# psipred/merizo_search

Hardware: AMD Instinct MI355X
Metric: queries/sec, exact 128-d cosine top-10 (recall@10 vs brute force = 1.0000) (higher is better)
Workload: dtype f32

## Files before the change

### merizo_search_amd/csrc/ms_scan_pf16.h

```cpp
#pragma once
#include "ms_scan_pf.h"

typedef _Float16 f16x8 __attribute__((ext_vector_type(8)));
constexpr uint32_t MS_PF16_MAGIC = 0x3631464du;
#define MS_PF_ERR_F16X2 5.5e-4f
#define MS_PF_ERR_F16X1 1.05e-3f

template <int KL, int NW, bool SAMPLE, bool MASK, int NQP>
__global__ __launch_bounds__(64 * NW, NW / 4) void ms_scan_pf16_kernel(const ScanParams p) {
    static_assert(NQP == 1 || NQP == 2, "query parts");
    static_assert(NW == 4 || NW == 8, "one or two waves per SIMD");
    constexpr int PPW = 16 / NW;
#ifdef MS_STAMP
    const unsigned long long tl_entry = __builtin_amdgcn_s_memrealtime();
    unsigned long long tl_setup = 0, tl_first = 0, tl_loop = 0;
#endif
    if (ms_gate_closed(p.gate, p.gate_epoch)) return;
    extern __shared__ __attribute__((aligned(16))) char smem[];
    typedef __attribute__((address_space(3))) char lds_char_t;
    typedef volatile __attribute__((address_space(3))) uint32_t lds_flag_t;
    typedef __attribute__((address_space(3))) ms_u32x2 lds_cand_t;
    const int tid = threadIdx.x, lane = tid & 63;
    const int wave = __builtin_amdgcn_readfirstlane(tid >> 6);
    const int r = lane & 31, h = lane >> 5;
    lds_flag_t *arrived = (lds_flag_t *)((lds_char_t *)smem + PF2_OFF_CNT);
    const float *auxring = reinterpret_cast<const float *>(smem + PF2_OFF_AUX);

    const int bid = blockIdx.x;
    const int per_super = 8 * p.n_qgroups;
    const int super = bid / per_super, within = bid % per_super;
    const int stream = super * 8 + (within & 7);
    const int qg = within >> 3;
    if (stream >= p.n_streams) return;
    const int64_t row_begin = (int64_t)stream * p.rows_per_stream;
    const int64_t row_end = (row_begin + p.rows_per_stream < p.n) ? row_begin + p.rows_per_stream : p.n;
    const int nfull = (int)((row_end - row_begin) >> 6);
    const int rem = (int)((row_end - row_begin) & 63);
    const int ntl = SAMPLE ? (nfull < p.max_tiles ? nfull : p.max_tiles) : nfull + (rem > 0 ? 1 : 0);
    constexpr bool mask_on = MASK;

    const int qtile = qg * NW + wave;
    const bool has_q = qtile < p.n_qtiles;
    if (tid < PF2_ARR) arrived[tid] = 0u;
    __syncthreads();
    const uint32_t ring_lds = __builtin_amdgcn_readfirstlane((uint32_t)(uintptr_t)(lds_char_t *)smem);

    const uint32_t voff = (uint32_t)(16 * lane);
    const uint64_t img0 = (uint64_t)(uintptr_t)p.pf_image + (uint64_t)(row_begin >> 6) * 16384u + (uint32_t)(1024 * PPW) * (uint32_t)wave;
    uint64_t it_sb = 0;
    uint32_t it_dst = 0;
    auto issue_prep = [&](int t) __attribute__((always_inline)) {
        const uint64_t b = img0 + (uint64_t)t * 16384u;
        const uint32_t b_lo = (uint32_t)__builtin_amdgcn_readfirstlane((uint32_t)b);
        const uint32_t b_hi = (uint32_t)__builtin_amdgcn_readfirstlane((uint32_t)(b >> 32));
        it_sb = ((uint64_t)b_hi << 32) | (uint64_t)b_lo;
        it_dst = (uint32_t)__builtin_amdgcn_readfirstlane(ring_lds + (uint32_t)(t % PF2_R) * 16384u + (uint32_t)(1024 * PPW) * (uint32_t)wave);
    };
    auto issue_piece = [&](auto i_c) __attribute__((always_inline)) {
        constexpr int I = decltype(i_c)::value;
        if constexpr (I < PPW) {
            const uint32_t d = (uint32_t)__builtin_amdgcn_readfirstlane(it_dst);
            const uint32_t lo = (uint32_t)__builtin_amdgcn_readfirstlane((uint32_t)it_sb), hi = (uint32_t)__builtin_amdgcn_readfirstlane((uint32_t)(it_sb >> 32));
            ms_glds_s16<1024 * I>(d + 1024 * I, voff, ((uint64_t)hi << 32) | (uint64_t)lo);
        }
    };
    auto issue_aux = [&](int t) __attribute__((always_inline)) {
        if constexpr (MASK) {
            int64_t row = row_begin + (int64_t)t * 64 + lane;
            if (row >= p.n) row = p.n - 1;
            const uint32_t dst = wave == 0 ? ring_lds + PF2_OFF_AUX + (uint32_t)(t % PF2_AUXR) * 256u
                                           : ring_lds + PF2_OFF_DUMMY + (uint32_t)(wave - 1) * 256u;
// ... 21 lines not shown
    auto read_arrived = [&](int t) __attribute__((always_inline)) { seen = arrived[t & (PF2_ARR - 1)]; };
    auto wait_arrived = [&](int t) __attribute__((always_inline)) {
        const uint32_t need = (uint32_t)NW * (uint32_t)(t / PF2_ARR + 1);
        uint32_t sv_, spins_, av_;
        static_assert(PF2_ARR == 16, "the mask below");
        asm volatile("s_waitcnt lgkmcnt(0)\n\t"
                     "v_readfirstlane_b32 %0, %2\n\t"
                     "s_cmp_ge_u32 %0, %5\n\t"
                     "s_setprio 2\n\t"
                     "s_cbranch_scc1 2f\n\t"
                     "s_setprio 0\n\t"
                     "s_and_b32 %0, %4, 15\n\t"
                     "s_lshl_b32 %0, %0, 2\n\t"
                     "s_add_u32 %0, %0, %6\n\t"
                     "v_mov_b32 %3, %0\n\t"
                     "s_mov_b32 %1, 0\n\t"
                     "1:\n\t"
                     "s_sleep 1\n\t"
                     "ds_read_b32 %2, %3\n\t"
                     "s_add_u32 %1, %1, 1\n\t"
                     "s_waitcnt lgkmcnt(0)\n\t"
                     "v_readfirstlane_b32 %0, %2\n\t"
                     "s_cmp_ge_u32 %0, %5\n\t"
                     "s_cbranch_scc1 2f\n\t"
                     "s_cmp_lt_u32 %1, 0x1000000\n\t"
                     "s_cbranch_scc1 1b\n\t"
                     "s_trap 2\n\t"
                     "2:"
                     : "=&s"(sv_), "=&s"(spins_), "+v"(seen), "=&v"(av_) : "s"(t), "s"(need), "s"(arr_lds) : "memory", "scc");
        asm volatile("" ::: "memory");
    };
    const int qidx = qtile * 32 + r;
    const bool q_valid = qidx < p.nq;
    const bool hist_on = !SAMPLE && p.hist != nullptr && p.lb_s != nullptr;
    f32x4 qv[16];
    float pre_lb = -INFINITY, pre_stp = 0.0f, pre_qlen = 0.0f;
    uint32_t pre_magic = MS_PF16_MAGIC, pre_n = (uint32_t)p.n;
    int pre_sr = 0;
    if (has_q) {
        const uint32_t *trailer = reinterpret_cast<const uint32_t *>(reinterpret_cast<const char *>(p.pf_image) + (size_t)((p.n + 63) >> 6) * 16384u);
        pre_magic = trailer[0];
        pre_sr = (int)trailer[1];
        pre_n = trailer[2];
        const f32x4 *src = reinterpret_cast<const f32x4 *>(p.qn + (size_t)(q_valid ? qidx : 0) * MS_DIM + 64 * h);
#pragma unroll
        for (int i = 0; i < 16; ++i) qv[i] = src[i];
        if (!SAMPLE && p.lb_s != nullptr) pre_lb = p.lb_s[qidx];
        if (hist_on && q_valid) pre_stp = p.hstep[qidx];
        if (MASK && p.qlen != nullptr && q_valid) pre_qlen = p.qlen[qidx];
    }
    asm volatile("" ::: "memory");
#pragma unroll
    for (int t = 0; t < PF2_D; ++t)
        if (t < ntl) issue_tile(t);

    if (!has_q) {
        if (ntl > 0) {
            if (ntl >= PF2_D) wait_own(std::integral_constant<int, PF2_D - PF2_W>{}); else ms_pf2_vmcnt<0>();
#pragma unroll
            for (int t = 0; t < PF2_W; ++t)
                if (t < ntl) publish(t);
        }
        for (int t = 0; t < ntl; ++t) {
            if (t + 1 < ntl) { read_arrived(t + 1); wait_arrived(t + 1); }
            if (t + PF2_D < ntl) {
                issue_tile(t + PF2_D);
                wait_own(std::integral_constant<int, PF2_D - PF2_W>{});
            } else {
                ms_pf2_vmcnt<0>();
            }
            if (t + PF2_W < ntl) publish(t + PF2_W);
        }
        return;
    }

    ScanState<SAMPLE ? 1 : KL> st;
    ScanHist hg;
    f16x8 qh[8], ql[NQP == 2 ? 8 : 1];
#pragma unroll
    for (int j = 0; j < (SAMPLE ? 1 : KL); ++j) { st.ls[j] = -INFINITY; st.li[j] = MS_IDX_NONE; }
    st.floor = -INFINITY;
    st.tau = -INFINITY;
    if (!SAMPLE && p.lb_s != nullptr) {
        const float lb = pre_lb;
        st.floor = (lb == -INFINITY) ? -INFINITY : nextafterf(lb, -INFINITY);
        st.tau = st.floor;
    }
    if (!q_valid) { st.floor = INFINITY; st.tau = INFINITY; }
    if (!SAMPLE && (p.debug_flags & 1)) { st.floor = INFINITY; st.tau = INFINITY; }
    hg.counters = nullptr; hg.base = 0.0f; hg.step = 0.0f; hg.inv_step = 0.0f;
    if (hist_on && q_valid) {
        const float stp = pre_stp, lb = pre_lb;
        if (stp > 0.0f && lb > -INFINITY) { hg.counters = p.hist + (size_t)qidx * 16; hg.base = lb; hg.step = stp; hg.inv_step = 1.0f / stp; }
    }
    float up = 1.0f, down = 1.0f;
    {
        const uint32_t magic = (uint32_t)__builtin_amdgcn_readfirstlane((int)pre_magic);
        const int sr = __builtin_amdgcn_readfirstlane(pre_sr);
        const uint32_t img_n = (uint32_t)__builtin_amdgcn_readfirstlane((int)pre_n);
        if (magic != MS_PF16_MAGIC || img_n != (uint32_t)p.n) __builtin_trap();
        f32x4 v[16];
        float m = 0.0f;
        float rinv = 1.0f;
        if (p.qraw_eps > 0.0f) {
            float ss = 0.0f;
#pragma unroll
            for (int i = 0; i < 16; ++i) { ss += qv[i].x * qv[i].x; ss += qv[i].y * qv[i].y; ss += qv[i].z * qv[i].z; ss += qv[i].w * qv[i].w; }
            ss = ss + ms_xor32_f(ss, h);
            rinv = 1.0f / fmaxf(sqrtf(ss), p.qraw_eps);
        }
#pragma unroll
        for (int i = 0; i < 16; ++i) {
            v[i] = q_valid ? qv[i] * rinv : f32x4{0.0f, 0.0f, 0.0f, 0.0f};
            m = fmaxf(m, fmaxf(fmaxf(fabsf(v[i].x), fabsf(v[i].y)), fmaxf(fabsf(v[i].z), fabsf(v[i].w))));
        }
        m = fmaxf(m, ms_xor32_f(m, h));
        int sq = 0;
        if (m > 0.0f && m < INFINITY) sq = 13 - ((int)((__float_as_uint(m) >> 23) & 0xFFu) - 127);
        sq = sq > 60 ? 60 : (sq < -60 ? -60 : sq);
        const float qs = __uint_as_float((uint32_t)(127 + sq) << 23);
        up = __uint_as_float((uint32_t)(127 + sr + sq) << 23);
        down = __uint_as_float((uint32_t)(127 - sr - sq) << 23);
#pragma unroll
        for (int b = 0; b < 8; ++b) {
            const f32x4 a0 = v[2 * b] * qs, a1 = v[2 * b + 1] * qs;
            const float x[8] = {a0.x, a0.y, a0.z, a0.w, a1.x, a1.y, a1.z, a1.w};
#pragma unroll
            for (int j = 0; j < 8; ++j) {
                const float c = fminf(fmaxf(x[j], -65504.0f), 65504.0f);
                const _Float16 hi16 = (_Float16)c;
                qh[b][j] = hi16;
                if constexpr (NQP == 2) ql[b][j] = (_Float16)(c - (float)hi16);
            }
        }
    }
    float tau_s = st.tau * up;
    const float my_qlen = (mask_on && p.qlen != nullptr && q_valid) ? pre_qlen : 0.0f;
    const float qlen_eff = mask_on ? my_qlen : INFINITY;
    const float mincov_eff = mask_on ? p.mincov : 0.0f;
    float smax = -INFINITY;
    auto apply_mask = [&](f32x16 &acc, int t, int half) __attribute__((always_inline)) {
        const f32x4 *ax = reinterpret_cast<const f32x4 *>(auxring + (t & (PF2_AUXR - 1)) * 64 + 32 * half + 4 * h);
#pragma unroll
        for (int g = 0; g < 4; ++g) {
            const f32x4 len4 = ax[2 * g];
#pragma unroll
            for (int j = 0; j < 4; ++j) {
                const float mk = (qlen_eff >= len4[j] * mincov_eff) ? 1.0f : 0.0f;
                acc[4 * g + j] = acc[4 * g + j] * mk;
            }
        }
    };
    bool neg_tau = !SAMPLE && mask_on && (__ballot(st.tau < 0.0f) != 0);
    const bool pace_on = !SAMPLE && p.prog != nullptr;
    constexpr int PACE_LEAD = 48;
    int pace_left = 16384;
    auto pace = [&](int t) __attribute__((always_inline)) {
        if (wave != 0 || (t & 15) != 0) return;
        const uint64_t line = (uint64_t)(uintptr_t)(p.prog + (size_t)stream * 16);
        const uint32_t l_lo = (uint32_t)__builtin_amdgcn_readfirstlane((uint32_t)line), l_hi = (uint32_t)__builtin_amdgcn_readfirstlane((uint32_t)(line >> 32));
        const uint64_t sline = ((uint64_t)l_hi << 32) | (uint64_t)l_lo;
        const uint32_t tag = p.prog_epoch << 24;
        if (lane == 0) __hip_atomic_store(p.prog + (size_t)stream * 16 + qg, tag | (uint32_t)t, __ATOMIC_RELAXED, __HIP_MEMORY_SCOPE_AGENT);
        if (t < PACE_LEAD) return;
        typedef uint32_t u32x16_ __attribute__((ext_vector_type(16)));
        for (; pace_left > 0; --pace_left) {
            u32x16_ w;
            asm volatile("s_load_dwordx16 %0, %1, 0x0 glc\n\ts_waitcnt lgkmcnt(0)" : "=s"(w) : "s"(sline) : "memory");
            uint32_t mn = 0xFFFFFFu;
#pragma unroll
            for (int i = 0; i < 16; ++i) {
                const uint32_t v = ((w[i] >> 24) == p.prog_epoch) ? (w[i] & 0xFFFFFFu) : 0u;
                if (i < p.n_qgroups) mn = v < mn ? v : mn;
            }
            if ((uint32_t)t <= mn + (uint32_t)PACE_LEAD) break;
            __builtin_amdgcn_s_sleep(64);
        }
    };
    auto retau = [&]() __attribute__((always_inline)) { tau_s = st.tau * up; };

    uint32_t ccnt = 0;
    auto cand_slot = [&](uint32_t c) __attribute__((always_inline)) -> lds_cand_t * {
        return (lds_cand_t *)((lds_char_t *)smem + PF2_OFF_CAND + (wave * PF2_CAND) * 512) + c * 64 + lane;
    };
    auto flush = [&]() __attribute__((always_inline)) {
        for (uint32_t c = 0; __ballot(ccnt > c) != 0; ++c) {
            const ms_u32x2 e = *cand_slot(c < PF2_CAND ? c : 0);
            const float v = (ccnt > c) ? __uint_as_float(e.x) : -INFINITY;
            ms_lane_insert<SAMPLE ? 1 : KL>(st, v, e.y, 0, h);
            ms_lane_insert<SAMPLE ? 1 : KL>(st, v, e.y, 1, h);
        }
        ccnt = 0;
        retau();
    };
    constexpr bool VISIT2 = !(MASK && (NQP == 2 || KL >= 16));
    auto visit_v2 = [&](f32x16 &sc_v, int t, int half, bool check_rows) __attribute__((always_inline)) {
        if (mask_on) apply_mask(sc_v, t, half);
        const uint32_t sub_row0 = (uint32_t)(row_begin + (int64_t)t * 64) + (uint32_t)(32 * half + 4 * h);
#pragma unroll 1
        for (;;) {
            bool ovf = false;
            float g0, g1, g2, g3;
            asm("v_max3_f32 %0, %4, %5, %6\n\tv_max3_f32 %1, %8, %9, %10\n\tv_max3_f32 %2, %12, %13, %14\n\tv_max3_f32 %3, %16, %17, %18\n\t"
                "v_max_f32 %0, %0, %7\n\tv_max_f32 %1, %1, %11\n\tv_max_f32 %2, %2, %15\n\tv_max_f32 %3, %3, %19"
                : "=&v"(g0), "=&v"(g1), "=&v"(g2), "=&v"(g3)
                : "v"(sc_v[0]), "v"(sc_v[1]), "v"(sc_v[2]), "v"(sc_v[3]), "v"(sc_v[4]), "v"(sc_v[5]), "v"(sc_v[6]), "v"(sc_v[7]), "v"(sc_v[8]),
                  "v"(sc_v[9]), "v"(sc_v[10]), "v"(sc_v[11]), "v"(sc_v[12]), "v"(sc_v[13]), "v"(sc_v[14]), "v"(sc_v[15]));
#define MS_PF16_REG(I)                                                                                                   \
            {                                                                                                            \
                const float ss = sc_v[I];                                                                                \
                const uint32_t row = sub_row0 + (uint32_t)(8 * ((I) >> 2) + ((I) & 3));                                    \
                bool pass = ss > tau_s;                                                                                  \
                if (check_rows) pass = pass && ((int64_t)row < row_end);                                                 \
                if (pass) {                                                                                              \
                    if (ccnt < (uint32_t)PF2_CAND) {                                                                     \
                        const float s_ = ss * down;                       \
                        if (hg.counters != nullptr) ms_hist_count(hg, s_);                                               \
                        *cand_slot(ccnt) = ms_u32x2{__float_as_uint(s_), row};                                           \
                        ccnt += 1;                                                                                       \
                        sc_v[I] = -INFINITY;                                                                             \
                    } else {                                                                                             \
                        ovf = true;                                                                                      \
                    }                                                                                                    \
// ... 42 lines not shown
            const uint32_t row = sub_row0 + (uint32_t)(8 * (i >> 2) + (i & 3));
            const float s = ss * down;
            bool pass = ss > tau_s;
            if (check_rows) pass = pass && ((int64_t)row < row_end);
            if (pass) {
                if (hg.counters != nullptr) ms_hist_count(hg, s);
                *cand_slot(ccnt) = ms_u32x2{__float_as_uint(s), row};
                ccnt += 1;
            }
            if (__builtin_expect(__ballot(ccnt >= PF2_CAND) != 0, 0)) flush();
        }
    };
    auto visit = [&](f32x16 &sc_v, int t, int half, bool check_rows) __attribute__((always_inline)) {
        if constexpr (VISIT2) visit_v2(sc_v, t, half, check_rows); else visit_v1(sc_v, t, half, check_rows);
    };

#ifdef MS_STAMP
    unsigned long long sp_t0 = 0, sp_sync = 0, sp_vis = 0, sp_nvis = 0, sp_chain = 0, sp_hist = 0, sp_lgkm = 0, sp_flow = 0;
#define PF2_T0() sp_t0 = __builtin_amdgcn_s_memtime()
#define PF2_ACC(V) { const unsigned long long now_ = __builtin_amdgcn_s_memtime(); V += now_ - sp_t0; sp_t0 = now_; }
#else
#define PF2_T0()
#define PF2_ACC(V)
#endif
    f32x4 fr[16];
    f32x16 acc0, acc1;
#pragma unroll
    for (int i = 0; i < 16; ++i) { acc0[i] = -INFINITY; acc1[i] = -INFINITY; }

    auto frag_base = [&](int t) __attribute__((always_inline)) -> const f32x4 * {
        return reinterpret_cast<const f32x4 *>(smem + (size_t)(t % PF2_R) * 16384 + 16 * lane);
    };
    auto filter = [&](int t, f32x16 &pv0, f32x16 &pv1) __attribute__((always_inline)) {
        if (SAMPLE) {
            if (mask_on && t > 0) { apply_mask(pv0, t - 1, 0); apply_mask(pv1, t - 1, 1); }
#pragma unroll
            for (int i = 0; i < 16; ++i) { smax = (pv0[i] > smax) ? pv0[i] : smax; smax = (pv1[i] > smax) ? pv1[i] : smax; }
        } else {
            float mx, mx1;
#define MS_PF16_MAX(M, PV)                                                                                                                        \
            asm("v_max3_f32 %0, %1, %2, %3\n\tv_max3_f32 %0, %0, %4, %5\n\tv_max3_f32 %0, %0, %6, %7\n\tv_max3_f32 %0, %0, %8, %9\n\t"             \
                "v_max3_f32 %0, %0, %10, %11\n\tv_max3_f32 %0, %0, %12, %13\n\tv_max3_f32 %0, %0, %14, %15\n\tv_max_f32 %0, %0, %16"               \
                : "=&v"(M) : "v"(PV[0]), "v"(PV[1]), "v"(PV[2]), "v"(PV[3]), "v"(PV[4]), "v"(PV[5]), "v"(PV[6]), "v"(PV[7]), "v"(PV[8]), "v"(PV[9]), \
                  "v"(PV[10]), "v"(PV[11]), "v"(PV[12]), "v"(PV[13]), "v"(PV[14]), "v"(PV[15]))
            MS_PF16_MAX(mx, pv0);
            MS_PF16_MAX(mx1, pv1);
#undef MS_PF16_MAX
            const bool hit0 = __ballot(mx > tau_s) != 0, hit1 = __ballot(mx1 > tau_s) != 0;
            if (__builtin_expect(hit0 || hit1 || neg_tau, 0)) {
                PF2_T0();
                if (t > 0) {
                    if (hit0 || neg_tau) visit(pv0, t - 1, 0, false);
                    if (hit1 || neg_tau) visit(pv1, t - 1, 1, false);
                }
                if (mask_on) neg_tau = __ballot(st.tau < 0.0f) != 0;
#ifdef MS_STAMP
                sp_nvis += 1;
#endif
                PF2_ACC(sp_vis)
            }
        }
    };
    auto stage = [&](auto steady_c, int t, f32x16 &out0, f32x16 &out1) __attribute__((always_inline)) {
        constexpr bool STEADY = decltype(steady_c)::value;
        PF2_T0();
        asm volatile("s_waitcnt lgkmcnt(0)" ::: "memory");
        PF2_ACC(sp_lgkm)
        if (STEADY || t + 1 < ntl) wait_arrived(t + 1);
        PF2_ACC(sp_sync)
        filter(t, out0, out1);
#pragma unroll
        for (int i = 0; i < 16; ++i) { out0[i] = 0.0f; out1[i] = 0.0f; }
        const f32x4 *src = frag_base(t + 1);
        const bool issuing = STEADY || t + PF2_D < ntl;
#define MS_PF2_BLOCK(B)                                                                                               \
        {                                                                                                             \
            const f16x8 f0 = __builtin_bit_cast(f16x8, fr[2 * (B)]), f1 = __builtin_bit_cast(f16x8, fr[2 * (B) + 1]);   \
            out0 = __builtin_amdgcn_mfma_f32_32x32x16_f16(f0, qh[B], out0, 0, 0, 0);                                  \
            out1 = __builtin_amdgcn_mfma_f32_32x32x16_f16(f1, qh[B], out1, 0, 0, 0);                                  \
            if constexpr (NQP == 2) {                                                                                 \
                out0 = __builtin_amdgcn_mfma_f32_32x32x16_f16(f0, ql[B], out0, 0, 0, 0);                              \
                out1 = __builtin_amdgcn_mfma_f32_32x32x16_f16(f1, ql[B], out1, 0, 0, 0);                              \
            }                                                                                                         \
            __builtin_amdgcn_sched_barrier(0);                                                                        \
            fr[2 * (B)] = src[64 * (2 * (B))];                                                                        \
            fr[2 * (B) + 1] = src[64 * (2 * (B) + 1)];                                                                \
        }
        MS_PF2_BLOCK(0)
        __builtin_amdgcn_sched_barrier(0);
        MS_PF2_BLOCK(1)
        if (STEADY || issuing) issue_prep(t + PF2_D);
        __builtin_amdgcn_sched_barrier(0);
        MS_PF2_BLOCK(2)
        if (STEADY || issuing) issue_piece(std::integral_constant<int, 0>{});
        __builtin_amdgcn_sched_barrier(0);
        MS_PF2_BLOCK(3)
        if (STEADY || issuing) issue_piece(std::integral_constant<int, 1>{});
        __builtin_amdgcn_sched_barrier(0);
        MS_PF2_BLOCK(4)
        if (STEADY || issuing) issue_piece(std::integral_constant<int, 2>{});
        __builtin_amdgcn_sched_barrier(0);
        MS_PF2_BLOCK(5)
        if (STEADY || issuing) { issue_piece(std::integral_constant<int, 3>{}); issue_aux(t + PF2_D); }
        __builtin_amdgcn_sched_barrier(0);
        MS_PF2_BLOCK(6)
        PF2_ACC(sp_chain)
        if (STEADY || issuing) wait_own(std::integral_constant<int, PF2_D - PF2_W>{}); else ms_pf2_vmcnt<0>();
        PF2_ACC(sp_flow)
        if (STEADY || t + PF2_W < ntl) publish(t + PF2_W);
        read_arrived(t + 2);
        __builtin_amdgcn_sched_barrier(0);
        MS_PF2_BLOCK(7)
#undef MS_PF2_BLOCK
#ifdef MS_STAMP
        asm volatile("s_nop 0" : "+v"(out0), "+v"(out1));
#endif
// ... 37 lines not shown
                PF2_T0();
                if (t - 1 + PF2_D < ntl) wait_own(std::integral_constant<int, 2>{}); else ms_pf2_vmcnt<0>();
                const ms_u32x4 *hp = reinterpret_cast<const ms_u32x4 *>(smem + PF2_OFF_HIST + hist_area * 2048 + r * 64);
                const ms_u32x4 c0 = hp[0], c1 = hp[1], c2 = hp[2], c3 = hp[3];
                const uint32_t c[16] = {c0.x, c0.y, c0.z, c0.w, c1.x, c1.y, c1.z, c1.w, c2.x, c2.y, c2.z, c2.w, c3.x, c3.y, c3.z, c3.w};
                uint32_t cum = 0;
                int n_lt = 0;
#pragma unroll
                for (int j = 15; j >= 0; --j) { cum += c[j]; n_lt += (cum < (uint32_t)p.k) ? 1 : 0; }
                const int J = 15 - n_lt;
                if (hg.counters != nullptr && J >= 1) {
                    st.floor = fmaxf(st.floor, ms_next_below(ms_hist_edge(hg, J)));
                    st.tau = fmaxf(st.tau, st.floor);
                }
                asm volatile("s_waitcnt lgkmcnt(0)" ::: "memory");
                retau();
                if (mask_on) neg_tau = __ballot(st.tau < 0.0f) != 0;
                PF2_ACC(sp_hist)
            }
        };
        int t = 0;
        for (; t + PF2_D < ntl; ++t) {
            if ((t & 1) == 0) {
                if (pace_on) pace(t);
                if (hist_on) hist_step(t);
            }
            stage(std::true_type{}, t, acc0, acc1);
        }
        for (; t < ntl; ++t) {
            if ((t & 1) == 0 && hist_on) hist_step(t);
            stage(std::false_type{}, t, acc0, acc1);
        }
#ifdef MS_STAMP
        if (!SAMPLE && lane == 0 && p.stamps != nullptr && (size_t)bid * 64 + 64 <= 4 * 4 * 65536) {
            unsigned long long *o = p.stamps + ((size_t)bid * 8 + wave) * 8;
            tl_loop = __builtin_amdgcn_s_memrealtime();
            o[0] = __builtin_amdgcn_s_memtime() - sp_c0;
            o[1] = __builtin_amdgcn_s_memrealtime() - sp_r0;
            o[2] = (unsigned long long)ntl;
            o[3] = (sp_lgkm << 32) | (sp_flow & 0xFFFFFFFFull);
            o[4] = sp_vis; o[5] = sp_nvis; o[6] = sp_chain; o[7] = (sp_hist << 32) | (sp_sync & 0xFFFFFFFFull);
        }
#endif
        if (pace_on && wave == 0 && lane == 0)
            __hip_atomic_store(p.prog + (size_t)stream * 16 + qg, (p.prog_epoch << 24) | 0xFFFFFFu, __ATOMIC_RELAXED, __HIP_MEMORY_SCOPE_AGENT);
        if (SAMPLE) {
            if (mask_on) { apply_mask(acc0, ntl - 1, 0); apply_mask(acc1, ntl - 1, 1); }
#pragma unroll
            for (int i = 0; i < 16; ++i) { smax = (acc0[i] > smax) ? acc0[i] : smax; smax = (acc1[i] > smax) ? acc1[i] : smax; }
        } else {
            visit(acc0, ntl - 1, 0, true);
            visit(acc1, ntl - 1, 1, true);
            flush();
        }
    }

    if (SAMPLE) {
        smax = smax * down;
        const float other = ms_xor32_f(smax, h);
        if (h == 0) {
            const float hi = (other > smax) ? other : smax, lo = (other > smax) ? smax : other;
            const size_t o = ((size_t)stream * p.nq_pad + qidx) * p.k;
            p.part_s[o] = hi;
            p.part_i[o] = (hi > -INFINITY) ? (uint32_t)(2 * stream) : MS_IDX_NONE;
            if (p.k > 1) {
                p.part_s[o + 1] = lo;
                p.part_i[o + 1] = (lo > -INFINITY) ? (uint32_t)(2 * stream + 1) : MS_IDX_NONE;
            }
        }
        return;
    }
#pragma unroll
    for (int j = 0; j < (SAMPLE ? 1 : KL); ++j) {
        const int rank = h * KL + j;
        if (rank < p.k) {
            const size_t o = ((size_t)stream * p.nq_pad + qidx) * p.k + rank;
            p.part_s[o] = st.ls[j];
            p.part_i[o] = st.li[j];
        }
    }
#ifdef MS_STAMP
    if (!SAMPLE && lane == 0 && p.stamps != nullptr && bid < 4096) {
        asm volatile("s_waitcnt vmcnt(0)" ::: "memory");
        unsigned long long *o = p.stamps + 8 * 8 * 4096 + ((size_t)bid * 8 + wave) * 8;
        o[0] = tl_entry; o[1] = tl_setup; o[2] = tl_first; o[3] = tl_loop; o[4] = __builtin_amdgcn_s_memrealtime();
    }
#endif
}

template <int KL, int NW, bool MASK, int NQP>
int launch_scan_pf16(const ScanPlan &pl, const ScanParams &sp, hipStream_t st) {
    MS_HIP_CHECK(hipFuncSetAttribute(reinterpret_cast<const void *>(ms_scan_pf16_kernel<KL, NW, false, MASK, NQP>),
                                     hipFuncAttributeMaxDynamicSharedMemorySize, (int)PF2_LDS));
    hipLaunchKernelGGL((ms_scan_pf16_kernel<KL, NW, false, MASK, NQP>), dim3(pl.d.grid), dim3(64 * NW), PF2_LDS, st, sp);
    MS_LAUNCH_CHECK("ms_scan_pf16_kernel");
    return MS_OK;
}
template <int KL, int NW>
int launch_scan_pf16_any(const ScanPlan &pl, const ScanParams &sp, hipStream_t st) {
    const bool two = sp.pf_format == MS_PF_F16X2;
    if (sp.lengths != nullptr) return two ? launch_scan_pf16<KL, NW, true, 2>(pl, sp, st) : launch_scan_pf16<KL, NW, true, 1>(pl, sp, st);
    return two ? launch_scan_pf16<KL, NW, false, 2>(pl, sp, st) : launch_scan_pf16<KL, NW, false, 1>(pl, sp, st);
}

int ms_launch_scan_pf16_kl5(const ScanPlan &pl, const ScanParams &sp, hipStream_t st);
int ms_launch_scan_pf16_kl10(const ScanPlan &pl, const ScanParams &sp, hipStream_t st);
int ms_launch_scan_pf16_kl16(const ScanPlan &pl, const ScanParams &sp, hipStream_t st);
int ms_launch_scan_pf16_kl32(const ScanPlan &pl, const ScanParams &sp, hipStream_t st);
int ms_launch_sample_pf16(const ScanPlan &pl, const ScanParams &sp, hipStream_t st);
int ms_launch_pf16_build_image(const float *db, int64_t n, int sr, void *image, hipStream_t st);
```

### merizo_search_amd/csrc/ms_scan_pf16_kl5.hip

```cpp
#include "ms_scan_pf16.h"

int ms_launch_scan_pf16_kl5(const ScanPlan &pl, const ScanParams &sp, hipStream_t st) {
    return sp.qpw == 2 ? launch_scan_pf16_any<5, 8>(pl, sp, st) : launch_scan_pf16_any<5, 4>(pl, sp, st);
}

template <int NW, bool MASK, int NQP>
static int launch_sample_pf16(const ScanPlan &pl, const ScanParams &sp, hipStream_t st) {
    MS_HIP_CHECK(hipFuncSetAttribute(reinterpret_cast<const void *>(ms_scan_pf16_kernel<5, NW, true, MASK, NQP>),
                                     hipFuncAttributeMaxDynamicSharedMemorySize, (int)PF2_LDS));
    hipLaunchKernelGGL((ms_scan_pf16_kernel<5, NW, true, MASK, NQP>), dim3(pl.d.grid), dim3(64 * NW), PF2_LDS, st, sp);
    MS_LAUNCH_CHECK("ms_scan_pf16_kernel (sample)");
    return MS_OK;
}
template <int NW>
static int launch_sample_pf16_any(const ScanPlan &pl, const ScanParams &sp, hipStream_t st) {
    const bool two = sp.pf_format == MS_PF_F16X2;
    if (sp.lengths != nullptr) return two ? launch_sample_pf16<NW, true, 2>(pl, sp, st) : launch_sample_pf16<NW, true, 1>(pl, sp, st);
    return two ? launch_sample_pf16<NW, false, 2>(pl, sp, st) : launch_sample_pf16<NW, false, 1>(pl, sp, st);
}

int ms_launch_sample_pf16(const ScanPlan &pl, const ScanParams &sp, hipStream_t st) {
    return sp.qpw == 2 ? launch_sample_pf16_any<8>(pl, sp, st) : launch_sample_pf16_any<4>(pl, sp, st);
}

__global__ __launch_bounds__(256) void ms_pf16_build_image_kernel(const float *db, int64_t n, char *image, int64_t ntiles, int sr) {
    const int lane = threadIdx.x & 63, r = lane & 31, h = lane >> 5;
    const float scale = __uint_as_float((uint32_t)(127 + sr) << 23);
    for (int64_t U = (int64_t)blockIdx.x * 4 + (threadIdx.x >> 6); U < 2 * ntiles; U += (int64_t)gridDim.x * 4) {
        const int64_t T = U >> 1;
        const int half = (int)(U & 1);
        const int64_t row = T * 64 + 32 * half + r;
        f32x4 x[16];
#pragma unroll
        for (int t = 0; t < 16; ++t) {
            x[t] = f32x4{0.0f, 0.0f, 0.0f, 0.0f};
            if (row < n) x[t] = *reinterpret_cast<const f32x4 *>(db + row * MS_DIM + 64 * h + 4 * t);
        }
        char *dst = image + T * 16384 + 16 * lane;
#pragma unroll
        for (int b = 0; b < 8; ++b) {
            const f32x4 a0 = x[2 * b] * scale, a1 = x[2 * b + 1] * scale;
            const float v[8] = {a0.x, a0.y, a0.z, a0.w, a1.x, a1.y, a1.z, a1.w};
            f16x8 o;
#pragma unroll
// ... 26 lines not shown
```

Baseline: 484,900.

## Split sample pass into dedicated double-buffered kernel with barrier-based tile staging

```diff
diff --git a/merizo_search_amd/csrc/ms_scan_pf16.h b/merizo_search_amd/csrc/ms_scan_pf16.h
--- a/merizo_search_amd/csrc/ms_scan_pf16.h
+++ b/merizo_search_amd/csrc/ms_scan_pf16.h
@@ -6,8 +6,77 @@
 #define MS_PF_ERR_F16X2 5.5e-4f
 #define MS_PF_ERR_F16X1 1.05e-3f
 
+__device__ __forceinline__ int ms_pf16_check_trailer(uint32_t pre_magic, int pre_sr, uint32_t pre_n, int64_t n) {
+    const uint32_t magic = (uint32_t)__builtin_amdgcn_readfirstlane((int)pre_magic);
+    const int sr = __builtin_amdgcn_readfirstlane(pre_sr);
+    const uint32_t img_n = (uint32_t)__builtin_amdgcn_readfirstlane((int)pre_n);
+    if (magic != MS_PF16_MAGIC || img_n != (uint32_t)n) __builtin_trap();
+    return sr;
+}
+template <int NQP>
+__device__ __forceinline__ void ms_pf16_prepare_query(const f32x4 (&qv)[16], bool q_valid, int h, float qraw_eps, int sr, f16x8 (&qh)[8],
+                                                      f16x8 (&ql)[NQP == 2 ? 8 : 1], float &up, float &down) {
+    f32x4 v[16];
+    float m = 0.0f;
+    float rinv = 1.0f;
+    if (qraw_eps > 0.0f) {
+        float ss = 0.0f;
+#pragma unroll
+        for (int i = 0; i < 16; ++i) { ss += qv[i].x * qv[i].x; ss += qv[i].y * qv[i].y; ss += qv[i].z * qv[i].z; ss += qv[i].w * qv[i].w; }
+        ss = ss + ms_xor32_f(ss, h);
+        rinv = 1.0f / fmaxf(sqrtf(ss), qraw_eps);
+    }
+#pragma unroll
+    for (int i = 0; i < 16; ++i) {
+        v[i] = q_valid ? qv[i] * rinv : f32x4{0.0f, 0.0f, 0.0f, 0.0f};
+        m = fmaxf(m, fmaxf(fmaxf(fabsf(v[i].x), fabsf(v[i].y)), fmaxf(fabsf(v[i].z), fabsf(v[i].w))));
+    }
+    m = fmaxf(m, ms_xor32_f(m, h));
+    int sq = 0;
+    if (m > 0.0f && m < INFINITY) sq = 13 - ((int)((__float_as_uint(m) >> 23) & 0xFFu) - 127);
+    sq = sq > 60 ? 60 : (sq < -60 ? -60 : sq);
+    const float qs = __uint_as_float((uint32_t)(127 + sq) << 23);
+    up = __uint_as_float((uint32_t)(127 + sr + sq) << 23);
+    down = __uint_as_float((uint32_t)(127 - sr - sq) << 23);
+#pragma unroll
+    for (int b = 0; b < 8; ++b) {
+        const f32x4 a0 = v[2 * b] * qs, a1 = v[2 * b + 1] * qs;
+        const float x[8] = {a0.x, a0.y, a0.z, a0.w, a1.x, a1.y, a1.z, a1.w};
+#pragma unroll
+        for (int j = 0; j < 8; ++j) {
+            const float c = fminf(fmaxf(x[j], -65504.0f), 65504.0f);
+            const _Float16 hi16 = (_Float16)c;
+            qh[b][j] = hi16;
+            if constexpr (NQP == 2) ql[b][j] = (_Float16)(c - (float)hi16);
+        }
+    }
+}
+template <int NQP>
+__device__ __forceinline__ void ms_pf16_block(const f32x4 &fa, const f32x4 &fb, const f16x8 &qh_b, const f16x8 &ql_b, f32x16 &out0, f32x16 &out1) {
+    const f16x8 f0 = __builtin_bit_cast(f16x8, fa), f1 = __builtin_bit_cast(f16x8, fb);
+    out0 = __builtin_amdgcn_mfma_f32_32x32x16_f16(f0, qh_b, out0, 0, 0, 0);
+    out1 = __builtin_amdgcn_mfma_f32_32x32x16_f16(f1, qh_b, out1, 0, 0, 0);
+    if constexpr (NQP == 2) {
+        out0 = __builtin_amdgcn_mfma_f32_32x32x16_f16(f0, ql_b, out0, 0, 0, 0);
+        out1 = __builtin_amdgcn_mfma_f32_32x32x16_f16(f1, ql_b, out1, 0, 0, 0);
+    }
+}
+__device__ __forceinline__ void ms_pf16_apply_mask(f32x16 &acc, const float *aux64, int half, int h, float qlen_eff, float mincov_eff) {
+    const f32x4 *ax = reinterpret_cast<const f32x4 *>(aux64 + 32 * half + 4 * h);
+#pragma unroll
+    for (int g = 0; g < 4; ++g) {
+        const f32x4 len4 = ax[2 * g];
+#pragma unroll
+        for (int j = 0; j < 4; ++j) {
+            const float mk = (qlen_eff >= len4[j] * mincov_eff) ? 1.0f : 0.0f;
+            acc[4 * g + j] = acc[4 * g + j] * mk;
+        }
+    }
+}
+
 template <int KL, int NW, bool SAMPLE, bool MASK, int NQP>
 __global__ __launch_bounds__(64 * NW, NW / 4) void ms_scan_pf16_kernel(const ScanParams p) {
+    static_assert(!SAMPLE, "the sample pass is ms_sample_pf16_kernel");
     static_assert(NQP == 1 || NQP == 2, "query parts");
     static_assert(NW == 4 || NW == 8, "one or two waves per SIMD");
     constexpr int PPW = 16 / NW;
@@ -36,7 +105,7 @@
     const int64_t row_end = (row_begin + p.rows_per_stream < p.n) ? row_begin + p.rows_per_stream : p.n;
     const int nfull = (int)((row_end - row_begin) >> 6);
     const int rem = (int)((row_end - row_begin) & 63);
-    const int ntl = SAMPLE ? (nfull < p.max_tiles ? nfull : p.max_tiles) : nfull + (rem > 0 ? 1 : 0);
+    const int ntl = nfull + (rem > 0 ? 1 : 0);
     constexpr bool mask_on = MASK;
 
     const int qtile = qg * NW + wave;
@@ -124,7 +193,7 @@
     };
     const int qidx = qtile * 32 + r;
     const bool q_valid = qidx < p.nq;
-    const bool hist_on = !SAMPLE && p.hist != nullptr && p.lb_s != nullptr;
+    const bool hist_on = p.hist != nullptr && p.lb_s != nullptr;
     f32x4 qv[16];
     float pre_lb = -INFINITY, pre_stp = 0.0f, pre_qlen = 0.0f;
     uint32_t pre_magic = MS_PF16_MAGIC, pre_n = (uint32_t)p.n;
@@ -137,7 +206,7 @@
         const f32x4 *src = reinterpret_cast<const f32x4 *>(p.qn + (size_t)(q_valid ? qidx : 0) * MS_DIM + 64 * h);
 #pragma unroll
         for (int i = 0; i < 16; ++i) qv[i] = src[i];
-        if (!SAMPLE && p.lb_s != nullptr) pre_lb = p.lb_s[qidx];
+        if (p.lb_s != nullptr) pre_lb = p.lb_s[qidx];
         if (hist_on && q_valid) pre_stp = p.hstep[qidx];
         if (MASK && p.qlen != nullptr && q_valid) pre_qlen = p.qlen[qidx];
     }
@@ -166,85 +235,36 @@
         return;
     }
 
-    ScanState<SAMPLE ? 1 : KL> st;
+    ScanState<KL> st;
     ScanHist hg;
     f16x8 qh[8], ql[NQP == 2 ? 8 : 1];
 #pragma unroll
-    for (int j = 0; j < (SAMPLE ? 1 : KL); ++j) { st.ls[j] = -INFINITY; st.li[j] = MS_IDX_NONE; }
+    for (int j = 0; j < KL; ++j) { st.ls[j] = -INFINITY; st.li[j] = MS_IDX_NONE; }
     st.floor = -INFINITY;
     st.tau = -INFINITY;
-    if (!SAMPLE && p.lb_s != nullptr) {
+    if (p.lb_s != nullptr) {
         const float lb = pre_lb;
         st.floor = (lb == -INFINITY) ? -INFINITY : nextafterf(lb, -INFINITY);
         st.tau = st.floor;
     }
     if (!q_valid) { st.floor = INFINITY; st.tau = INFINITY; }
-    if (!SAMPLE && (p.debug_flags & 1)) { st.floor = INFINITY; st.tau = INFINITY; }
+    if (p.debug_flags & 1) { st.floor = INFINITY; st.tau = INFINITY; }
     hg.counters = nullptr; hg.base = 0.0f; hg.step = 0.0f; hg.inv_step = 0.0f;
     if (hist_on && q_valid) {
         const float stp = pre_stp, lb = pre_lb;
         if (stp > 0.0f && lb > -INFINITY) { hg.counters = p.hist + (size_t)qidx * 16; hg.base = lb; hg.step = stp; hg.inv_step = 1.0f / stp; }
     }
     float up = 1.0f, down = 1.0f;
-    {
-        const uint32_t magic = (uint32_t)__builtin_amdgcn_readfirstlane((int)pre_magic);
-        const int sr = __builtin_amdgcn_readfirstlane(pre_sr);
-        const uint32_t img_n = (uint32_t)__builtin_amdgcn_readfirstlane((int)pre_n);
-        if (magic != MS_PF16_MAGIC || img_n != (uint32_t)p.n) __builtin_trap();
-        f32x4 v[16];
-        float m = 0.0f;
-        float rinv = 1.0f;
-        if (p.qraw_eps > 0.0f) {
-            float ss = 0.0f;
-#pragma unroll
-            for (int i = 0; i < 16; ++i) { ss += qv[i].x * qv[i].x; ss += qv[i].y * qv[i].y; ss += qv[i].z * qv[i].z; ss += qv[i].w * qv[i].w; }
-            ss = ss + ms_xor32_f(ss, h);
-            rinv = 1.0f / fmaxf(sqrtf(ss), p.qraw_eps);
-        }
-#pragma unroll
-        for (int i = 0; i < 16; ++i) {
-            v[i] = q_valid ? qv[i] * rinv : f32x4{0.0f, 0.0f, 0.0f, 0.0f};
-            m = fmaxf(m, fmaxf(fmaxf(fabsf(v[i].x), fabsf(v[i].y)), fmaxf(fabsf(v[i].z), fabsf(v[i].w))));
-        }
-        m = fmaxf(m, ms_xor32_f(m, h));
-        int sq = 0;
-        if (m > 0.0f && m < INFINITY) sq = 13 - ((int)((__float_as_uint(m) >> 23) & 0xFFu) - 127);
-        sq = sq > 60 ? 60 : (sq < -60 ? -60 : sq);
-        const float qs = __uint_as_float((uint32_t)(127 + sq) << 23);
-        up = __uint_as_float((uint32_t)(127 + sr + sq) << 23);
-        down = __uint_as_float((uint32_t)(127 - sr - sq) << 23);
-#pragma unroll
-        for (int b = 0; b < 8; ++b) {
-            const f32x4 a0 = v[2 * b] * qs, a1 = v[2 * b + 1] * qs;
-            const float x[8] = {a0.x, a0.y, a0.z, a0.w, a1.x, a1.y, a1.z, a1.w};
-#pragma unroll
-            for (int j = 0; j < 8; ++j) {
-                const float c = fminf(fmaxf(x[j], -65504.0f), 65504.0f);
-                const _Float16 hi16 = (_Float16)c;
-                qh[b][j] = hi16;
-                if constexpr (NQP == 2) ql[b][j] = (_Float16)(c - (float)hi16);
-            }
-        }
-    }
+    ms_pf16_prepare_query<NQP>(qv, q_valid, h, p.qraw_eps, ms_pf16_check_trailer(pre_magic, pre_sr, pre_n, p.n), qh, ql, up, down);
     float tau_s = st.tau * up;
     const float my_qlen = (mask_on && p.qlen != nullptr && q_valid) ? pre_qlen : 0.0f;
     const float qlen_eff = mask_on ? my_qlen : INFINITY;
     const float mincov_eff = mask_on ? p.mincov : 0.0f;
-    float smax = -INFINITY;
     auto apply_mask = [&](f32x16 &acc, int t, int half) __attribute__((always_inline)) {
-        const f32x4 *ax = reinterpret_cast<const f32x4 *>(auxring + (t & (PF2_AUXR - 1)) * 64 + 32 * half + 4 * h);
-#pragma unroll
-        for (int g = 0; g < 4; ++g) {
-            const f32x4 len4 = ax[2 * g];
-#pragma unroll
-            for (int j = 0; j < 4; ++j) {
-                const float mk = (qlen_eff >= len4[j] * mincov_eff) ? 1.0f : 0.0f;
-                acc[4 * g + j] = acc[4 * g + j] * mk;
-            }
-        }
-    };
-    bool neg_tau = !SAMPLE && mask_on && (__ballot(st.tau < 0.0f) != 0);
-    const bool pace_on = !SAMPLE && p.prog != nullptr;
+        ms_pf16_apply_mask(acc, auxring + (t & (PF2_AUXR - 1)) * 64, half, h, qlen_eff, mincov_eff);
+    };
+    bool neg_tau = mask_on && (__ballot(st.tau < 0.0f) != 0);
+    const bool pace_on = p.prog != nullptr;
     constexpr int PACE_LEAD = 48;
     int pace_left = 16384;
     auto pace = [&](int t) __attribute__((always_inline)) {
@@ -279,8 +299,8 @@
         for (uint32_t c = 0; __ballot(ccnt > c) != 0; ++c) {
             const ms_u32x2 e = *cand_slot(c < PF2_CAND ? c : 0);
             const float v = (ccnt > c) ? __uint_as_float(e.x) : -INFINITY;
-            ms_lane_insert<SAMPLE ? 1 : KL>(st, v, e.y, 0, h);
-            ms_lane_insert<SAMPLE ? 1 : KL>(st, v, e.y, 1, h);
+            ms_lane_insert<KL>(st, v, e.y, 0, h);
+            ms_lane_insert<KL>(st, v, e.y, 1, h);
         }
         ccnt = 0;
         retau();
@@ -389,33 +409,27 @@
         return reinterpret_cast<const f32x4 *>(smem + (size_t)(t % PF2_R) * 16384 + 16 * lane);
     };
     auto filter = [&](int t, f32x16 &pv0, f32x16 &pv1) __attribute__((always_inline)) {
-        if (SAMPLE) {
-            if (mask_on && t > 0) { apply_mask(pv0, t - 1, 0); apply_mask(pv1, t - 1, 1); }
-#pragma unroll
-            for (int i = 0; i < 16; ++i) { smax = (pv0[i] > smax) ? pv0[i] : smax; smax = (pv1[i] > smax) ? pv1[i] : smax; }
-        } else {
-            float mx, mx1;
+        float mx, mx1;
 #define MS_PF16_MAX(M, PV)                                                                                                                        \
-            asm("v_max3_f32 %0, %1, %2, %3\n\tv_max3_f32 %0, %0, %4, %5\n\tv_max3_f32 %0, %0, %6, %7\n\tv_max3_f32 %0, %0, %8, %9\n\t"             \
-                "v_max3_f32 %0, %0, %10, %11\n\tv_max3_f32 %0, %0, %12, %13\n\tv_max3_f32 %0, %0, %14, %15\n\tv_max_f32 %0, %0, %16"               \
-                : "=&v"(M) : "v"(PV[0]), "v"(PV[1]), "v"(PV[2]), "v"(PV[3]), "v"(PV[4]), "v"(PV[5]), "v"(PV[6]), "v"(PV[7]), "v"(PV[8]), "v"(PV[9]), \
-                  "v"(PV[10]), "v"(PV[11]), "v"(PV[12]), "v"(PV[13]), "v"(PV[14]), "v"(PV[15]))
-            MS_PF16_MAX(mx, pv0);
-            MS_PF16_MAX(mx1, pv1);
+        asm("v_max3_f32 %0, %1, %2, %3\n\tv_max3_f32 %0, %0, %4, %5\n\tv_max3_f32 %0, %0, %6, %7\n\tv_max3_f32 %0, %0, %8, %9\n\t"             \
+            "v_max3_f32 %0, %0, %10, %11\n\tv_max3_f32 %0, %0, %12, %13\n\tv_max3_f32 %0, %0, %14, %15\n\tv_max_f32 %0, %0, %16"               \
+            : "=&v"(M) : "v"(PV[0]), "v"(PV[1]), "v"(PV[2]), "v"(PV[3]), "v"(PV[4]), "v"(PV[5]), "v"(PV[6]), "v"(PV[7]), "v"(PV[8]), "v"(PV[9]), \
+              "v"(PV[10]), "v"(PV[11]), "v"(PV[12]), "v"(PV[13]), "v"(PV[14]), "v"(PV[15]))
+        MS_PF16_MAX(mx, pv0);
+        MS_PF16_MAX(mx1, pv1);
 #undef MS_PF16_MAX
-            const bool hit0 = __ballot(mx > tau_s) != 0, hit1 = __ballot(mx1 > tau_s) != 0;
-            if (__builtin_expect(hit0 || hit1 || neg_tau, 0)) {
-                PF2_T0();
-                if (t > 0) {
-                    if (hit0 || neg_tau) visit(pv0, t - 1, 0, false);
-                    if (hit1 || neg_tau) visit(pv1, t - 1, 1, false);
-                }
-                if (mask_on) neg_tau = __ballot(st.tau < 0.0f) != 0;
+        const bool hit0 = __ballot(mx > tau_s) != 0, hit1 = __ballot(mx1 > tau_s) != 0;
+        if (__builtin_expect(hit0 || hit1 || neg_tau, 0)) {
+            PF2_T0();
+            if (t > 0) {
+                if (hit0 || neg_tau) visit(pv0, t - 1, 0, false);
+                if (hit1 || neg_tau) visit(pv1, t - 1, 1, false);
+            }
+            if (mask_on) neg_tau = __ballot(st.tau < 0.0f) != 0;
 #ifdef MS_STAMP
-                sp_nvis += 1;
+            sp_nvis += 1;
 #endif
-                PF2_ACC(sp_vis)
-            }
+            PF2_ACC(sp_vis)
         }
     };
     auto stage = [&](auto steady_c, int t, f32x16 &out0, f32x16 &out1) __attribute__((always_inline)) {
@@ -432,13 +446,7 @@
         const bool issuing = STEADY || t + PF2_D < ntl;
 #define MS_PF2_BLOCK(B)                                                                                               \
         {                                                                                                             \
-            const f16x8 f0 = __builtin_bit_cast(f16x8, fr[2 * (B)]), f1 = __builtin_bit_cast(f16x8, fr[2 * (B) + 1]);   \
-            out0 = __builtin_amdgcn_mfma_f32_32x32x16_f16(f0, qh[B], out0, 0, 0, 0);                                  \
-            out1 = __builtin_amdgcn_mfma_f32_32x32x16_f16(f1, qh[B], out1, 0, 0, 0);                                  \
-            if constexpr (NQP == 2) {                                                                                 \
-                out0 = __builtin_amdgcn_mfma_f32_32x32x16_f16(f0, ql[B], out0, 0, 0, 0);                              \
-                out1 = __builtin_amdgcn_mfma_f32_32x32x16_f16(f1, ql[B], out1, 0, 0, 0);                              \
-            }                                                                                                         \
+            ms_pf16_block<NQP>(fr[2 * (B)], fr[2 * (B) + 1], qh[B], ql[NQP == 2 ? (B) : 0], out0, out1);              \
             __builtin_amdgcn_sched_barrier(0);                                                                        \
             fr[2 * (B)] = src[64 * (2 * (B))];                                                                        \
             fr[2 * (B) + 1] = src[64 * (2 * (B) + 1)];                                                                \
@@ -542,7 +550,7 @@
             stage(std::false_type{}, t, acc0, acc1);
         }
 #ifdef MS_STAMP
-        if (!SAMPLE && lane == 0 && p.stamps != nullptr && (size_t)bid * 64 + 64 <= 4 * 4 * 65536) {
+        if (lane == 0 && p.stamps != nullptr && (size_t)bid * 64 + 64 <= 4 * 4 * 65536) {
             unsigned long long *o = p.stamps + ((size_t)bid * 8 + wave) * 8;
             tl_loop = __builtin_amdgcn_s_memrealtime();
             o[0] = __builtin_amdgcn_s_memtime() - sp_c0;
@@ -554,34 +562,13 @@
 #endif
         if (pace_on && wave == 0 && lane == 0)
             __hip_atomic_store(p.prog + (size_t)stream * 16 + qg, (p.prog_epoch << 24) | 0xFFFFFFu, __ATOMIC_RELAXED, __HIP_MEMORY_SCOPE_AGENT);
-        if (SAMPLE) {
-            if (mask_on) { apply_mask(acc0, ntl - 1, 0); apply_mask(acc1, ntl - 1, 1); }
-#pragma unroll
-            for (int i = 0; i < 16; ++i) { smax = (acc0[i] > smax) ? acc0[i] : smax; smax = (acc1[i] > smax) ? acc1[i] : smax; }
-        } else {
-            visit(acc0, ntl - 1, 0, true);
-            visit(acc1, ntl - 1, 1, true);
-            flush();
-        }
-    }
-
-    if (SAMPLE) {
-        smax = smax * down;
-        const float other = ms_xor32_f(smax, h);
-        if (h == 0) {
-            const float hi = (other > smax) ? other : smax, lo = (other > smax) ? smax : other;
-            const size_t o = ((size_t)stream * p.nq_pad + qidx) * p.k;
-            p.part_s[o] = hi;
-            p.part_i[o] = (hi > -INFINITY) ? (uint32_t)(2 * stream) : MS_IDX_NONE;
-            if (p.k > 1) {
-                p.part_s[o + 1] = lo;
-                p.part_i[o + 1] = (lo > -INFINITY) ? (uint32_t)(2 * stream + 1) : MS_IDX_NONE;
-            }
-        }
-        return;
-    }
-#pragma unroll
-    for (int j = 0; j < (SAMPLE ? 1 : KL); ++j) {
+        visit(acc0, ntl - 1, 0, true);
+        visit(acc1, ntl - 1, 1, true);
+        flush();
+    }
+
+#pragma unroll
+    for (int j = 0; j < KL; ++j) {
         const int rank = h * KL + j;
         if (rank < p.k) {
             const size_t o = ((size_t)stream * p.nq_pad + qidx) * p.k + rank;
@@ -590,7 +577,7 @@
         }
     }
 #ifdef MS_STAMP
-    if (!SAMPLE && lane == 0 && p.stamps != nullptr && bid < 4096) {
+    if (lane == 0 && p.stamps != nullptr && bid < 4096) {
         asm volatile("s_waitcnt vmcnt(0)" ::: "memory");
         unsigned long long *o = p.stamps + 8 * 8 * 4096 + ((size_t)bid * 8 + wave) * 8;
         o[0] = tl_entry; o[1] = tl_setup; o[2] = tl_first; o[3] = tl_loop; o[4] = __builtin_amdgcn_s_memrealtime();
@@ -613,6 +600,168 @@
     return two ? launch_scan_pf16<KL, NW, false, 2>(pl, sp, st) : launch_scan_pf16<KL, NW, false, 1>(pl, sp, st);
 }
 
+constexpr int PF16S_HALF = 4;
+constexpr int PF16S_OFF_AUX = 2 * PF16S_HALF * 16384;
+constexpr int PF16S_OFF_DUMMY = PF16S_OFF_AUX + 2 * PF16S_HALF * 256;
+constexpr int PF16S_LDS = PF16S_OFF_DUMMY + 7 * 256;
+static_assert(PF16S_LDS <= 160 * 1024, "LDS of one CU");
+
+template <int NW, bool MASK, int NQP>
+__global__ __launch_bounds__(64 * NW, NW / 4) void ms_sample_pf16_kernel(const ScanParams p) {
+    static_assert(NQP == 1 || NQP == 2, "query parts");
+    static_assert(NW == 4 || NW == 8, "one or two waves per SIMD");
+    constexpr int PPW = 16 / NW;
+    constexpr int PT = PPW + (MASK ? 1 : 0);
+    static_assert(PF16S_HALF * PT < 64, "vmcnt is a 6-bit counter");
+    if (ms_gate_closed(p.gate, p.gate_epoch)) return;
+    extern __shared__ __attribute__((aligned(16))) char smem[];
+    typedef __attribute__((address_space(3))) char lds_char_t;
+    const int tid = threadIdx.x, lane = tid & 63;
+    const int wave = __builtin_amdgcn_readfirstlane(tid >> 6);
+    const int r = lane & 31, h = lane >> 5;
+
+    const int bid = blockIdx.x;
+    const int per_super = 8 * p.n_qgroups;
+    const int super = bid / per_super, within = bid % per_super;
+    const int stream = super * 8 + (within & 7);
+    const int qg = within >> 3;
+    if (stream >= p.n_streams) return;
+    const int64_t row_begin = (int64_t)stream * p.rows_per_stream;
+    const int64_t row_end = (row_begin + p.rows_per_stream < p.n) ? row_begin + p.rows_per_stream : p.n;
+    const int nfull = (int)((row_end - row_begin) >> 6);
+    const int ntl = nfull < p.max_tiles ? nfull : p.max_tiles;
+    const int nh = (ntl + PF16S_HALF - 1) / PF16S_HALF;
+    auto tiles_of = [&](int c) __attribute__((always_inline)) -> int {
+        const int left = ntl - c * PF16S_HALF;
+        return left < 0 ? 0 : (left < PF16S_HALF ? left : PF16S_HALF);
+    };
+
+    const int qtile = qg * NW + wave;
+    const bool has_q = qtile < p.n_qtiles;
+    const uint32_t lds0 = __builtin_amdgcn_readfirstlane((uint32_t)(uintptr_t)(lds_char_t *)smem);
+
+    const int qidx = qtile * 32 + r;
+    const bool q_valid = qidx < p.nq;
+    f32x4 qv[16];
+    float pre_qlen = 0.0f;
+    uint32_t pre_magic = MS_PF16_MAGIC, pre_n = (uint32_t)p.n;
+    int pre_sr = 0;
+    if (has_q) {
+        const uint32_t *trailer = reinterpret_cast<const uint32_t *>(reinterpret_cast<const char *>(p.pf_image) + (size_t)((p.n + 63) >> 6) * 16384u);
+        pre_magic = trailer[0];
+        pre_sr = (int)trailer[1];
+        pre_n = trailer[2];
+        const f32x4 *src = reinterpret_cast<const f32x4 *>(p.qn + (size_t)(q_valid ? qidx : 0) * MS_DIM + 64 * h);
+#pragma unroll
+        for (int i = 0; i < 16; ++i) qv[i] = src[i];
+        if (MASK && p.qlen != nullptr && q_valid) pre_qlen = p.qlen[qidx];
+    }
+    asm volatile("" ::: "memory");
+
+    const uint32_t voff = (uint32_t)(16 * lane);
+    const uint64_t img0 = (uint64_t)(uintptr_t)p.pf_image + (uint64_t)(row_begin >> 6) * 16384u + (uint32_t)(1024 * PPW) * (uint32_t)wave;
+    auto issue_half = [&](int c) __attribute__((always_inline)) {
+        const int nt = tiles_of(c);
+#pragma unroll
+        for (int j = 0; j < PF16S_HALF; ++j) {
+            if (j < nt) {
+                const int t = c * PF16S_HALF + j;
+                const int slot = (c & 1) * PF16S_HALF + j;
+                const uint64_t b = img0 + (uint64_t)t * 16384u;
+                const uint32_t b_lo = (uint32_t)__builtin_amdgcn_readfirstlane((uint32_t)b);
+                const uint32_t b_hi = (uint32_t)__builtin_amdgcn_readfirstlane((uint32_t)(b >> 32));
+                const uint64_t sb = ((uint64_t)b_hi << 32) | (uint64_t)b_lo;
+                const uint32_t d = (uint32_t)__builtin_amdgcn_readfirstlane(lds0 + (uint32_t)slot * 16384u + (uint32_t)(1024 * PPW) * (uint32_t)wave);
+                ms_glds_s16<0>(d, voff, sb);
+                ms_glds_s16<1024>(d + 1024, voff, sb);
+                if constexpr (PPW == 4) {
+                    ms_glds_s16<2048>(d + 2048, voff, sb);
+                    ms_glds_s16<3072>(d + 3072, voff, sb);
+                }
+                if constexpr (MASK) {
+                    int64_t row = row_begin + (int64_t)t * 64 + lane;
+                    if (row >= p.n) row = p.n - 1;
+                    const uint32_t dst = wave == 0 ? lds0 + PF16S_OFF_AUX + (uint32_t)slot * 256u : lds0 + PF16S_OFF_DUMMY + (uint32_t)(wave - 1) * 256u;
+                    ms_glds_v4((uint32_t)__builtin_amdgcn_readfirstlane(dst), p.lengths + row);
+                }
+            }
+        }
+    };
+    auto wait_but = [&](int young) __attribute__((always_inline)) {
+        if (young <= 0) ms_pf2_vmcnt<0>();
+        else if (young == 1) ms_pf2_vmcnt<PT>();
+        else if (young == 2) ms_pf2_vmcnt<2 * PT>();
+        else if (young == 3) ms_pf2_vmcnt<3 * PT>();
+        else ms_pf2_vmcnt<4 * PT>();
+    };
+    static_assert(PF16S_HALF == 4, "wait_but");
+    auto barrier = [&]() __attribute__((always_inline)) { asm volatile("s_waitcnt lgkmcnt(0)\n\ts_barrier" ::: "memory"); };
+
+    if (nh > 0) issue_half(0);
+    if (nh > 1) issue_half(1);
+
+    f16x8 qh[8], ql[NQP == 2 ? 8 : 1];
+    float up = 1.0f, down = 1.0f;
+    if (has_q) ms_pf16_prepare_query<NQP>(qv, q_valid, h, p.qraw_eps, ms_pf16_check_trailer(pre_magic, pre_sr, pre_n, p.n), qh, ql, up, down);
+    const float qlen_eff = MASK ? ((p.qlen != nullptr && q_valid) ? pre_qlen : 0.0f) : INFINITY;
+    const float mincov_eff = MASK ? p.mincov : 0.0f;
+    float smax = -INFINITY;
+
+    auto scan_half = [&](int buf, int nt) __attribute__((always_inline)) {
+        const char *base = smem + (size_t)buf * (PF16S_HALF * 16384) + 16 * lane;
+        const float *aux = reinterpret_cast<const float *>(smem + PF16S_OFF_AUX) + buf * (PF16S_HALF * 64);
+        f32x4 fr[16];
+        {
+            const f32x4 *src = reinterpret_cast<const f32x4 *>(base);
+#pragma unroll
+            for (int f = 0; f < 16; ++f) fr[f] = src[64 * f];
+        }
+#pragma unroll 1
+        for (int t = 0; t < nt; ++t) {
+            const f32x4 *nx = reinterpret_cast<const f32x4 *>(base + (size_t)(t + 1 < nt ? t + 1 : t) * 16384);
+            f32x16 a0, a1;
+#pragma unroll
+            for (int i = 0; i < 16; ++i) { a0[i] = 0.0f; a1[i] = 0.0f; }
+#pragma unroll
+            for (int b = 0; b < 8; ++b) {
+                ms_pf16_block<NQP>(fr[2 * b], fr[2 * b + 1], qh[b], ql[NQP == 2 ? b : 0], a0, a1);
+                fr[2 * b] = nx[64 * (2 * b)];
+                fr[2 * b + 1] = nx[64 * (2 * b + 1)];
+            }
+            if constexpr (MASK) {
+                ms_pf16_apply_mask(a0, aux + t * 64, 0, h, qlen_eff, mincov_eff);
+                ms_pf16_apply_mask(a1, aux + t * 64, 1, h, qlen_eff, mincov_eff);
+            }
+#pragma unroll
+            for (int i = 0; i < 16; ++i) { smax = (a0[i] > smax) ? a0[i] : smax; smax = (a1[i] > smax) ? a1[i] : smax; }
+        }
+    };
+
+    for (int c = 0; c < nh; ++c) {
+        wait_but(tiles_of(c + 1));
+        barrier();
+        if (has_q) scan_half(c & 1, tiles_of(c));
+        if (c + 2 < nh) {
+            barrier();
+            issue_half(c + 2);
+        }
+    }
+    if (!has_q) return;
+
+    smax = smax * down;
+    const float other = ms_xor32_f(smax, h);
+    if (h == 0) {
+        const float hi = (other > smax) ? other : smax, lo = (other > smax) ? smax : other;
+        const size_t o = ((size_t)stream * p.nq_pad + qidx) * p.k;
+        p.part_s[o] = hi;
+        p.part_i[o] = (hi > -INFINITY) ? (uint32_t)(2 * stream) : MS_IDX_NONE;
+        if (p.k > 1) {
+            p.part_s[o + 1] = lo;
+            p.part_i[o + 1] = (lo > -INFINITY) ? (uint32_t)(2 * stream + 1) : MS_IDX_NONE;
+        }
+    }
+}
+
 int ms_launch_scan_pf16_kl5(const ScanPlan &pl, const ScanParams &sp, hipStream_t st);
 int ms_launch_scan_pf16_kl10(const ScanPlan &pl, const ScanParams &sp, hipStream_t st);
 int ms_launch_scan_pf16_kl16(const ScanPlan &pl, const ScanParams &sp, hipStream_t st);
diff --git a/merizo_search_amd/csrc/ms_scan_pf16_kl5.hip b/merizo_search_amd/csrc/ms_scan_pf16_kl5.hip
--- a/merizo_search_amd/csrc/ms_scan_pf16_kl5.hip
+++ b/merizo_search_amd/csrc/ms_scan_pf16_kl5.hip
@@ -6,10 +6,10 @@
 
 template <int NW, bool MASK, int NQP>
 static int launch_sample_pf16(const ScanPlan &pl, const ScanParams &sp, hipStream_t st) {
-    MS_HIP_CHECK(hipFuncSetAttribute(reinterpret_cast<const void *>(ms_scan_pf16_kernel<5, NW, true, MASK, NQP>),
-                                     hipFuncAttributeMaxDynamicSharedMemorySize, (int)PF2_LDS));
-    hipLaunchKernelGGL((ms_scan_pf16_kernel<5, NW, true, MASK, NQP>), dim3(pl.d.grid), dim3(64 * NW), PF2_LDS, st, sp);
-    MS_LAUNCH_CHECK("ms_scan_pf16_kernel (sample)");
+    MS_HIP_CHECK(hipFuncSetAttribute(reinterpret_cast<const void *>(ms_sample_pf16_kernel<NW, MASK, NQP>),
+                                     hipFuncAttributeMaxDynamicSharedMemorySize, (int)PF16S_LDS));
+    hipLaunchKernelGGL((ms_sample_pf16_kernel<NW, MASK, NQP>), dim3(pl.d.grid), dim3(64 * NW), PF16S_LDS, st, sp);
+    MS_LAUNCH_CHECK("ms_sample_pf16_kernel");
     return MS_OK;
 }
 template <int NW>
```

After: 484,600. No clear change (-0.1%).
